# juanmc2005/diart

Measured on AMD Instinct MI355X. Metric: real-time-factor xRT streams/GPU @500ms step, higher is better.
Workload: dtype f16x3

## Files before the change

### diart_amd/csrc/k_mlp_head.hip

```cpp
#include "dz_common.h"

namespace {

typedef _Float16 f16x8 __attribute__((ext_vector_type(8)));
typedef _Float16 f16x4 __attribute__((ext_vector_type(4)));
typedef float f32x16 __attribute__((ext_vector_type(16)));

constexpr int PLANE = 128 * 64;
constexpr int R0 = 0, R1 = 8 * PLANE;
constexpr int M1_PITCH = 129;
constexpr int PAR = R1 + 128 * M1_PITCH * 4 + 64;
constexpr int PAR_B0 = 0, PAR_B1 = 128, PAR_CW = 256, PAR_CB = 256 + 8 * 128;
constexpr size_t LDS_BYTES = PAR + (PAR_CB + 8) * sizeof(float);
constexpr float LO_UNSCALE = 1.f / 2048.f;

__device__ __forceinline__ float leaky(float v) { return v > 0.f ? v : v * DZ_LEAKY_SLOPE; }

__global__ __launch_bounds__(256) void mlp_head_kernel(DzMlpHead p) {
    extern __shared__ __attribute__((aligned(16))) char smem[];
    const int tid = threadIdx.x;
    const int w = __builtin_amdgcn_readfirstlane(tid >> 6), l = tid & 63;
    const int t0 = blockIdx.x * 128;

    float* par = reinterpret_cast<float*>(smem + PAR);
    if (tid < 128) {
        par[PAR_B0 + tid] = p.b0[tid];
        par[PAR_B1 + tid] = p.b1[tid];
    }
    for (int i = tid; i < p.classes * 128; i += 256) par[PAR_CW + i] = p.cw[i];
    if (tid < p.classes) par[PAR_CB + tid] = p.cb[tid];

    const bool isB = w >= 2;
    const int lo = w & 1;
    const unsigned short* A = reinterpret_cast<const unsigned short*>(p.Xsplit);
    const unsigned short* W0 = reinterpret_cast<const unsigned short*>(p.W0split);
    const unsigned short* W1 = reinterpret_cast<const unsigned short*>(p.W1split);
    const unsigned short* src = isB ? W0 + (long long)lo * 128 * 256 : A + (long long)lo * p.xplane;
    const unsigned nbytes = (unsigned)((isB ? 128ll : (long long)p.rows) * 256 * 2);
    const __amdgpu_buffer_rsrc_t rsrc = __builtin_amdgcn_make_buffer_rsrc((void*)src, 0, nbytes, 0x00020000);
    const int chunk = ((l & 3) ^ ((l >> 4) & 3)) << 4;
    const int voff0 = ((isB ? 0 : t0) + (l >> 2)) * 64 + chunk;
    const int kb_bytes = (isB ? 128 : p.rows) * 64;
    auto issue0 = [&](int kt, int stage) {
        char* dst = smem + R0 + stage * 4 * PLANE + w * PLANE;
#pragma unroll
        for (int i = 0; i < 8; ++i)
            __builtin_amdgcn_raw_ptr_buffer_load_lds(
                rsrc, (__attribute__((address_space(3))) void*)(dst + i * 1024), 16, voff0 + i * 1024, kt * kb_bytes, 0, 0);
    };
    const __amdgpu_buffer_rsrc_t rs1 = __builtin_amdgcn_make_buffer_rsrc((void*)W1, 0, 2u * 128 * 128 * 2, 0x00020000);
    auto issue1 = [&]() {
        const int voff1 = (l >> 2) * 64 + chunk;
#pragma unroll
        for (int pl = 0; pl < 2; ++pl)
#pragma unroll
            for (int i = 0; i < 8; ++i)
                __builtin_amdgcn_raw_ptr_buffer_load_lds(
                    rs1, (__attribute__((address_space(3))) void*)(smem + R0 + w * 2 * PLANE + pl * PLANE + i * 1024), 16,
                    voff1 + i * 1024 + pl * (128 * 128 * 2), w * (128 * 64), 0, 0);
    };

    const int li = l & 31, g = l >> 5;
    const int wm = w >> 1, wn = w & 1;
    const int sw = (li >> 2) & 3;
    int foff[2];
#pragma unroll
    for (int ks = 0; ks < 2; ++ks) foff[ks] = li * 64 + (((2 * ks + g) ^ sw) << 4);
    f32x16 accm[2][2], accx[2][2];
    auto zero = [&]() {
#pragma unroll
        for (int mt = 0; mt < 2; ++mt)
#pragma unroll
            for (int nt = 0; nt < 2; ++nt)
#pragma unroll
                for (int r = 0; r < 16; ++r) accm[mt][nt][r] = accx[mt][nt][r] = 0.f;
    };
    auto compute = [&](const char* a_hi, const char* b_hi) {
        const char* sa = a_hi + (wm * 64) * 64;
        const char* sb = b_hi + (wn * 64) * 64;
#pragma unroll
        for (int ks = 0; ks < 2; ++ks) {
            f16x8 ah[2], al[2], bh[2], bl[2];
#pragma unroll
            for (int t = 0; t < 2; ++t) {
                ah[t] = *reinterpret_cast<const f16x8*>(sa + t * 2048 + foff[ks]);
                al[t] = *reinterpret_cast<const f16x8*>(sa + PLANE + t * 2048 + foff[ks]);
                bh[t] = *reinterpret_cast<const f16x8*>(sb + t * 2048 + foff[ks]);
                bl[t] = *reinterpret_cast<const f16x8*>(sb + PLANE + t * 2048 + foff[ks]);
            }
#pragma unroll
            for (int mt = 0; mt < 2; ++mt)
#pragma unroll
                for (int nt = 0; nt < 2; ++nt) {
                    accx[mt][nt] = __builtin_amdgcn_mfma_f32_32x32x16_f16(bh[nt], al[mt], accx[mt][nt], 0, 0, 0);
                    accm[mt][nt] = __builtin_amdgcn_mfma_f32_32x32x16_f16(bh[nt], ah[mt], accm[mt][nt], 0, 0, 0);
                    accx[mt][nt] = __builtin_amdgcn_mfma_f32_32x32x16_f16(bl[nt], ah[mt], accx[mt][nt], 0, 0, 0);
                }
        }
    };

    zero();
    issue0(0, 0);
    for (int kt = 0; kt < 8; ++kt) {
        asm volatile("s_waitcnt vmcnt(0) lgkmcnt(0)\n\ts_barrier" ::: "memory");
        if (kt + 1 < 8) issue0(kt + 1, (kt + 1) & 1);
        const char* st = smem + R0 + (kt & 1) * 4 * PLANE;
        compute(st, st + 2 * PLANE);
    }
    asm volatile("s_waitcnt lgkmcnt(0)\n\ts_barrier" ::: "memory");
    issue1();

    float amax = 0.f;
#pragma unroll
    for (int mt = 0; mt < 2; ++mt) {
        const int row = wm * 64 + mt * 32 + li;
#pragma unroll
        for (int nt = 0; nt < 2; ++nt)
#pragma unroll
            for (int k = 0; k < 4; ++k) {
                const int n = wn * 64 + nt * 32 + 8 * k + 4 * g;
                const f32x4 bv = *reinterpret_cast<const f32x4*>(par + PAR_B0 + n);
                f32x4 v;
#pragma unroll
                for (int e = 0; e < 4; ++e) {
                    float x = leaky((accm[mt][nt][4 * k + e] + accx[mt][nt][4 * k + e] * LO_UNSCALE) + bv[e]);
                    amax = fmaxf(amax, fabsf(x));
                    v[e] = __builtin_amdgcn_fmed3f(x, -65504.f, 65504.f);
                }
                const f16x4 hi = __builtin_convertvector(v, f16x4);
                const f16x4 lo4 = __builtin_convertvector((v - __builtin_convertvector(hi, f32x4)) * 2048.f, f16x4);
                char* d = smem + R1 + (wn * 2 + nt) * 2 * PLANE + row * 64 + ((k ^ ((row >> 2) & 3)) << 4) + 8 * g;
                *reinterpret_cast<f16x4*>(d) = hi;
                *reinterpret_cast<f16x4*>(d + PLANE) = lo4;
            }
    }
    dz_flag_range(p.oflag, amax);

    zero();
    asm volatile("s_waitcnt vmcnt(0) lgkmcnt(0)\n\ts_barrier" ::: "memory");
#pragma unroll
    for (int kt = 0; kt < 4; ++kt) compute(smem + R1 + kt * 2 * PLANE, smem + R0 + kt * 2 * PLANE);
    asm volatile("s_waitcnt lgkmcnt(0)\n\ts_barrier" ::: "memory");

    float* m1 = reinterpret_cast<float*>(smem + R1);
#pragma unroll
    for (int mt = 0; mt < 2; ++mt) {
        const int row = wm * 64 + mt * 32 + li;
#pragma unroll
        for (int nt = 0; nt < 2; ++nt)
#pragma unroll
            for (int k = 0; k < 4; ++k) {
                const int n = wn * 64 + nt * 32 + 8 * k + 4 * g;
                const f32x4 bv = *reinterpret_cast<const f32x4*>(par + PAR_B1 + n);
#pragma unroll
                for (int e = 0; e < 4; ++e)
                    m1[row * M1_PITCH + n + e] =
                        leaky((accm[mt][nt][4 * k + e] + accx[mt][nt][4 * k + e] * LO_UNSCALE) + bv[e]);
            }
    }
    __syncthreads();

    const int t = t0 + tid;
    if (tid < 128 && t < p.rows) {
        const float* x = m1 + tid * M1_PITCH;
        float lg[8];
        for (int c = 0; c < p.classes; ++c) {
            float acc = 0.f;
            const float* wc = par + PAR_CW + c * 128;
#pragma unroll 8
            for (int k = 0; k < 128; ++k) acc = fmaf(x[k], wc[k], acc);
            lg[c] = acc + par[PAR_CB + c];
        }
        float s[8];
        dz_seg_decide(lg, p.classes, p.K, p.powerset, s);
        const int b = t / p.F, f = t - b * p.F;
        if (p.wave_mom && dz_ws_bad(p.wave_mom, b))
            for (int k = 0; k < p.K; ++k) s[k] = __builtin_nanf("");
        for (int k = 0; k < p.K; ++k) p.seg[(long long)t * p.K + k] = s[k];
        if (p.wout) {
            float wv[8];
            dz_osp_frame(s, p.K, p.gamma, p.beta, wv);
            for (int k = 0; k < p.K; ++k) p.wout[((long long)b * p.K + k) * p.F + f] = wv[k];
        }
    }
}

}

int dz_launch_mlp_head(const DzMlpHead& p_in, hipStream_t st) {
    DzMlpHead p = p_in;
    if (!p.oflag) p.oflag = dz_cur_oflag;
    DZ_REQUIRE(p.Xsplit && p.W0split && p.W1split && p.b0 && p.b1 && p.cw && p.cb && p.seg, "mlp_head: NULL argument");
    DZ_REQUIRE(p.rows > 0 && p.F > 0 && p.rows % p.F == 0, "mlp_head: %d rows are not whole chunks of %d frames", p.rows, p.F);
    DZ_REQUIRE(p.classes >= 1 && p.classes <= 8 && p.K >= 1 && p.K <= 8 && (p.powerset || p.K == p.classes),
               "mlp_head: classes %d / speakers %d", p.classes, p.K);
    DZ_REQUIRE((long long)p.rows * 256 * 2 < (1ll << 31), "mlp_head: plane exceeds the buffer range");
    DZ_REQUIRE(p.xplane == (long long)p.rows * 256, "mlp_head: kb-major input planes of exactly `rows` rows (xplane = rows * 256)");
    static DzAttrOnce attr_once;
    DZ_HIP(attr_once.raise((const void*)mlp_head_kernel, (int)LDS_BYTES));
    DZ_LAUNCH(mlp_head_kernel, dim3((p.rows + 127) / 128), dim3(256), LDS_BYTES, st, p);
    DZ_HIP(hipGetLastError());
    return 0;
}
```

Measured before the change: 33650.

## Deepen MLP head load pipeline to four stages and parallelize classifier

The K-loop staging goes from double buffering to a four-slot ring with three tile loads in flight. Partial vmcnt waits let compute overlap several outstanding buffer-to-LDS loads, and the extra stages reuse LDS that the later m1 buffer occupies. The final classifier dot products now use all 256 threads, each computing four classes per frame with vectorized weight reads. Logits pass through shared memory, which costs an extra barrier, and weights are zero-padded to 8 classes.

```diff
diff --git a/diart_amd/csrc/k_mlp_head.hip b/diart_amd/csrc/k_mlp_head.hip
--- a/diart_amd/csrc/k_mlp_head.hip
+++ b/diart_amd/csrc/k_mlp_head.hip
@@ -27,7 +27,7 @@
         par[PAR_B0 + tid] = p.b0[tid];
         par[PAR_B1 + tid] = p.b1[tid];
     }
-    for (int i = tid; i < p.classes * 128; i += 256) par[PAR_CW + i] = p.cw[i];
+    for (int i = tid; i < 8 * 128; i += 256) par[PAR_CW + i] = i < p.classes * 128 ? p.cw[i] : 0.f;
     if (tid < p.classes) par[PAR_CB + tid] = p.cb[tid];
 
     const bool isB = w >= 2;
@@ -100,11 +100,15 @@
     };
 
     zero();
-    issue0(0, 0);
+#pragma unroll
+    for (int s = 0; s < 3; ++s) issue0(s, s);
+#pragma unroll 1
     for (int kt = 0; kt < 8; ++kt) {
-        asm volatile("s_waitcnt vmcnt(0) lgkmcnt(0)\n\ts_barrier" ::: "memory");
-        if (kt + 1 < 8) issue0(kt + 1, (kt + 1) & 1);
-        const char* st = smem + R0 + (kt & 1) * 4 * PLANE;
+        if (kt < 6) asm volatile("s_waitcnt vmcnt(16) lgkmcnt(0)\n\ts_barrier" ::: "memory");
+        else if (kt == 6) asm volatile("s_waitcnt vmcnt(8) lgkmcnt(0)\n\ts_barrier" ::: "memory");
+        else asm volatile("s_waitcnt vmcnt(0) lgkmcnt(0)\n\ts_barrier" ::: "memory");
+        if (kt + 3 < 8) issue0(kt + 3, (kt + 3) & 3);
+        const char* st = smem + R0 + (kt & 3) * 4 * PLANE;
         compute(st, st + 2 * PLANE);
     }
     asm volatile("s_waitcnt lgkmcnt(0)\n\ts_barrier" ::: "memory");
@@ -160,17 +164,33 @@
     }
     __syncthreads();
 
+    {
+        const int fr = tid & 127, c0 = (tid >> 7) * 4;
+        const float* x = m1 + fr * M1_PITCH;
+        const float* wc = par + PAR_CW + c0 * 128;
+        float acc[4] = {0.f, 0.f, 0.f, 0.f};
+#pragma unroll 2
+        for (int k = 0; k < 128; k += 4) {
+            float xk[4];
+#pragma unroll
+            for (int j = 0; j < 4; ++j) xk[j] = x[k + j];
+#pragma unroll
+            for (int c = 0; c < 4; ++c) {
+                const f32x4 wv = *reinterpret_cast<const f32x4*>(wc + c * 128 + k);
+#pragma unroll
+                for (int j = 0; j < 4; ++j) acc[c] = fmaf(xk[j], wv[j], acc[c]);
+            }
+        }
+        float* lgs = reinterpret_cast<float*>(smem + R0) + fr * 9;
+#pragma unroll
+        for (int c = 0; c < 4; ++c)
+            if (c0 + c < p.classes) lgs[c0 + c] = acc[c] + par[PAR_CB + c0 + c];
+    }
+    __syncthreads();
     const int t = t0 + tid;
     if (tid < 128 && t < p.rows) {
-        const float* x = m1 + tid * M1_PITCH;
         float lg[8];
-        for (int c = 0; c < p.classes; ++c) {
-            float acc = 0.f;
-            const float* wc = par + PAR_CW + c * 128;
-#pragma unroll 8
-            for (int k = 0; k < 128; ++k) acc = fmaf(x[k], wc[k], acc);
-            lg[c] = acc + par[PAR_CB + c];
-        }
+        for (int c = 0; c < p.classes; ++c) lg[c] = reinterpret_cast<const float*>(smem + R0)[tid * 9 + c];
         float s[8];
         dz_seg_decide(lg, p.classes, p.K, p.powerset, s);
         const int b = t / p.F, f = t - b * p.F;
```

Result: no change. 33820, median of 6 (+0.5%).
